# Rudrabha/Wav2Lip

Measured on AMD Instinct MI355X. Metric: face-frames/sec (96x96, mel T=16), higher is better.
Workload: dtype f32

## Files before the change

include/w2l_hip.h:

```cpp
#ifndef W2L_HIP_H
#define W2L_HIP_H

#include <stddef.h>
#include <stdint.h>

#ifdef __cplusplus
extern "C" {
#endif

#define W2L_OK 0
#define W2L_ERR_ARG (-1)
#define W2L_ERR_HIP (-2)
#define W2L_ERR_NOMEM (-3)

#define W2L_ACT_NONE 0
#define W2L_ACT_RELU 1
#define W2L_ACT_SIGMOID 2
#define W2L_ACT_LEAKY 3

#define W2L_PREC_F32 0
#define W2L_PREC_BF16 1

const char* w2l_last_error(void);
int w2l_abi_version(void);
// ... 198 lines not shown
int w2l_thin1x1_dgrad_bf16(void* stream, long long npix, int cin, int cout, const void* dz, int dz_cs, const float* w,
                           const void* res, int res_cs, void* dx, int dx_cs);
int w2l_thin1x1_wgrad_bf16(void* stream, long long npix, int cin, int cout, const void* x, int x_cs, const void* dz, int dz_cs,
                           float* dweight, float* dbias);
int w2l_thin1x1_wgrad_blocks(long long npix);
int w2l_nchw_to_nhwc_bf16(void* stream, int N, int C, int H, int W, const float* x, void* y, int y_cs, int c_zero_to);
int w2l_nhwc_bf16_to_nchw(void* stream, int N, int C, int H, int W, const void* x, int x_cs, float* y);


int w2l_bn_train_stats(void* stream, long long rows, int C, const float* z, int z_cs, const float* gamma,
                       const float* beta, float eps, float momentum, float* running_mean, float* running_var,
                       float* mean, float* rstd, float* scale, float* shift);
int w2l_affine_act(void* stream, long long rows, int C, const float* z, int z_cs, const float* scale,
                   const float* shift, const float* res, int res_cs, int act, float* y, int y_cs);
int w2l_bn_train_bwd(void* stream, long long rows, int C, const float* dy, int dy_cs, const float* y, int y_cs,
                     const float* z, int z_cs, int act, const float* mean, const float* rstd, const float* scale,
                     float* dgamma, float* dbeta, float* dz, int dz_cs, float* g_out, int g_cs);
int w2l_act_bwd(void* stream, long long rows, int C, const float* dy, int dy_cs, const float* y, int y_cs, int act,
                const float* scale, float* dz, int dz_cs, float* g_out, int g_cs);
int w2l_add_rows(void* stream, long long rows, int C, const float* a, int a_cs, const float* b, int b_cs, float* out,
                 int out_cs);
int w2l_col_sum(void* stream, long long rows, int C, const float* x, int x_cs, float* out);

int w2l_l1_mean(void* stream, long long n, const float* a, const float* b, float* loss_out);
int w2l_l1_bwd(void* stream, long long n, const float* a, const float* b, const float* gout, float* da);
int w2l_cosine_bce_bwd(void* stream, int N, int C, const float* a, const float* v, const float* y, const float* gout,
                       float* da, float* dv);
int w2l_l2norm_bwd(void* stream, int N, int C, const float* x, int x_cs, const float* dy, float* dx, int dx_cs);
int w2l_bce_bwd(void* stream, int N, const float* p, const float* y, const float* gout, float* dp);

int w2l_shifted_pdist(void* stream, int T, int C, int vshift, const float* f1, const float* f2, float* out);

typedef struct {
    uint64_t frames, mel;
    int32_t T, start;
    int32_t pad[2];
} w2l_sync_row;
typedef struct {
    int32_t row0, n;
} w2l_lse_segment;

int w2l_sync_window_rows(void* stream, int B, const w2l_sync_row* rows, int S, float* face_in, int face_cs, float* mel_in,
                         int mel_cs);
int w2l_lse_score_segments(void* stream, int n_seg, const w2l_lse_segment* segs, int C, int vshift, const float* face_emb,
                           const float* audio_emb, float* mdist, float* scores);

typedef struct w2l_adam_tensor {
    float* param;
    const float* grad;
    float* exp_avg;
    float* exp_avg_sq;
    long long n;
} w2l_adam_tensor;
typedef struct w2l_adam w2l_adam_t;
int w2l_adam_create(int ntensors, const long long* sizes_host, w2l_adam_t** out);
int w2l_adam_destroy(w2l_adam_t* h);
int w2l_adam_step(w2l_adam_t* h, void* stream, const w2l_adam_tensor* tensors_host, float lr, float beta1, float beta2,
                  float eps, float weight_decay, int step);


typedef struct w2l_plan w2l_plan_t;
int w2l_plan_create(w2l_plan_t** out);
int w2l_plan_destroy(w2l_plan_t* p);
int w2l_plan_add_conv(w2l_plan_t* p, const w2l_conv_t* c, int N, int H, int W, const float* x, int x_cs,
                      float* y, int y_cs, const float* res, int res_cs);
int w2l_plan_add_convb(w2l_plan_t* p, const w2l_convb_t* c, int N, int H, int W, const void* x, int x_cs, void* y, int y_cs,
                       const void* res, int res_cs, const float* scale, const float* shift);
int w2l_plan_add_convb_head(w2l_plan_t* p, const w2l_convb_t* c, int N, int H, int W, const void* x, int x_cs, uint8_t* frames,
                            float* y32, int y32_cs, const float* scale, const float* shift);
int w2l_plan_copy_item(w2l_plan_t* dst, const w2l_plan_t* src, int index);
int w2l_plan_run(const w2l_plan_t* p, void* stream);
int w2l_plan_size(const w2l_plan_t* p);
int w2l_plan_autotune(w2l_plan_t* p, void* stream, int reps);
int w2l_plan_get_config(const w2l_plan_t* p, int index, int* tile, int* ksplit);
int w2l_plan_set_config(w2l_plan_t* p, int index, int tile, int ksplit);
int w2l_plan_executed_flops(const w2l_plan_t* p, long long* flops_out, int* config_out);
int w2l_conv_num_igemm_tiles(void);
int w2l_flops_begin(void);
long long w2l_flops_end(long long* by_family);
int w2l_clock_probe(void* stream, int spin_us, unsigned long long* out2_dev);
int w2l_conv_config_family(int id);
int w2l_conv_exclude_families(int mask);
int w2l_igemm_block_order(int order, int order_r, int tiles_m, int tiles_n, int nphase, int* out);
int w2l_plan_profile(const w2l_plan_t* p, void* stream, int reps, float* ms_out);

#define W2L_TUNE_KEY_INTS 17
int w2l_tune_key_ints(void);
int w2l_tune_set(const int* key, int tile, int ksplit);
int w2l_tune_entry_applicable(const int* key, int tile);
int w2l_tune_clear(void);
int w2l_tune_count(void);
int w2l_tune_export(int* out, int cap_entries);

#ifdef __cplusplus
}
#endif
#endif
```

wav2lip_amd/_lib.py:

```python
import ctypes as C
import os

_HERE = os.path.dirname(os.path.abspath(__file__))
LIB_PATH = os.environ.get("W2L_HIP_LIB") or os.path.join(_HERE, "lib", "libw2l_hip.so")

ACT_NONE, ACT_RELU, ACT_SIGMOID, ACT_LEAKY = 0, 1, 2, 3
PREC_F32, PREC_BF16 = 0, 1


class ConvGeom(C.Structure):
    _fields_ = [(n, C.c_int) for n in
                ("transposed", "cin", "cout", "kh", "kw", "sh", "sw", "ph", "pw", "oph", "opw", "act")]


class AdamTensor(C.Structure):
    _fields_ = [("param", C.c_void_p), ("grad", C.c_void_p), ("exp_avg", C.c_void_p), ("exp_avg_sq", C.c_void_p),
                ("n", C.c_longlong)]


class WgradInfo(C.Structure):
    _fields_ = [(n, C.c_int) for n in ("family", "cfg", "ksplit", "chunk", "K", "kstep", "reduce_blocks")]


class WgradBf16Info(C.Structure):
# ... 72 lines not shown
    "w2l_mel_create": (_i, [_vp, _vp, C.POINTER(_vp)]),
    "w2l_mel_destroy": (_i, [_vp]),
    "w2l_mel_num_frames": (_i, [_ll]),
    "w2l_melspectrogram": (_i, [_vp, _vp, _vp, _ll, _vp]),
    "w2l_mel_stream_cols": (_i, [_vp, _vp, _vp, _i, _vp, _i]),
    "w2l_mel_gather": (_i, [_vp, _vp, _i, _vp, _i, _vp, _i, _i]),
    "w2l_mel_gather_bf16": (_i, [_vp, _vp, _i, _vp, _i, _vp, _i, _i]),
    "w2l_mel_gather_rows": (_i, [_vp, _vp, _i, _vp, _i, _i]),
    "w2l_mel_gather_rows_bf16": (_i, [_vp, _vp, _i, _vp, _i, _i]),
    "w2l_resample_sinc": (_i, [_vp, _vp, _i, _vp, _i, C.c_double, _vp, _vp, _i, _i, _vp]),
    "w2l_l2norm_rows": (_i, [_vp, _i, _i, _vp, _i, _vp]),
    "w2l_cosine_bce": (_i, [_vp, _i, _i, _vp, _vp, _vp, _vp, _vp]),
    "w2l_bce_mean": (_i, [_vp, _i, _vp, _vp, _vp]),
    "w2l_conv_update": (_i, [_vp, _vp, _vp, _vp, _vp]),
    "w2l_conv_wgrad": (_i, [C.POINTER(ConvGeom), _vp, _i, _i, _i, _vp, _i, _vp, _i, _vp]),
    "w2l_conv_wgrad_prec": (_i, [C.POINTER(ConvGeom), _vp, _i, _i, _i, _vp, _i, _vp, _i, _vp, _i]),
    "w2l_conv_wgrad_resolve": (_i, [C.POINTER(ConvGeom), _i, _i, _i, _i, _i, _i, C.POINTER(WgradInfo)]),
    "w2l_conv_wgrad_set_cfg": (_i, [_i, _i]),
    "w2l_wgrad_divmod_host": (_i, [_i, _i, _vp, _vp, _vp, _vp]),
    "w2l_convb_create": (_i, [C.POINTER(ConvGeom), _vp, _vp, C.POINTER(_vp)]),
    "w2l_convb_update": (_i, [_vp, _vp, _vp]),
    "w2l_convb_update_many": (_i, [_i, _vp, _vp, _vp]),
    "w2l_convb_destroy": (_i, [_vp]),
    "w2l_convb_forward": (_i, [_vp, _vp, _i, _i, _i, _vp, _i, _vp, _i, _vp, _i, _vp, _vp, _i]),
    "w2l_convb_attach_head": (_i, [_vp, _vp, _vp, _vp, _i, _i, _vp]),
    "w2l_convb_forward_head": (_i, [_vp, _vp, _i, _i, _i, _vp, _i, _vp, _vp, _i, _vp, _vp]),
    "w2l_convb_forward_bn": (_i, [_vp, _vp, _i, _i, _i, _vp, _i, _vp, _i, _vp, _vp, _vp, _f, _f, _vp, _vp, _vp, _vp, _vp, _vp]),
    "w2l_convb_forward_bnbwd": (_i, [_vp, _vp, _i, _i, _i, _vp, _i, _vp, _i, _vp, _i, _vp, _i, _vp, _i, _i, _vp, _vp, _vp, _vp, _vp, _vp,
                                     C.POINTER(C.c_int)]),
    "w2l_convb_forward_actbwd": (_i, [_vp, _vp, _i, _i, _i, _vp, _i, _vp, _i, _vp, _i, _vp, _i, _i, _vp, C.POINTER(C.c_int)]),
    "w2l_convb_set_tile": (_i, [_vp, _i]),
    "w2l_convb_num_tiles": (_i, []),
    "w2l_convb_resolve": (_i, [_vp, _i, _i, _i, _i, C.POINTER(C.c_int), C.POINTER(C.c_int), C.POINTER(C.c_int)]),
    "w2l_conv_wgrad_bf16": (_i, [C.POINTER(ConvGeom), _vp, _i, _i, _i, _vp, _i, _vp, _i, _vp]),
    "w2l_conv_wgrad_bf16_resolve": (_i, [C.POINTER(ConvGeom), _i, _i, _i, _i, _i, C.POINTER(WgradBf16Info)]),
    "w2l_bn_train_stats_bf16": (_i, [_vp, _ll, _i, _i, _vp, _i, _vp, _vp, _f, _f, _vp, _vp, _vp, _vp, _vp, _vp]),
    "w2l_affine_act_bf16": (_i, [_vp, _ll, _i, _vp, _i, _vp, _vp, _vp, _i, _i, _vp, _i]),
    "w2l_bn_train_bwd_bf16": (_i, [_vp, _ll, _i, _i, _vp, _i, _vp, _i, _vp, _i, _i, _vp, _vp, _vp, _vp, _vp, _vp, _vp, _i, _vp, _i]),
    "w2l_bn_train_bwd_apply_bf16": (_i, [_vp, _ll, _i, _vp, _i, _vp, _i, _vp, _i, _i, _vp, _vp, _vp, _vp, _vp, _vp, _vp, _i, _vp, _i]),
    "w2l_act_bwd_bf16": (_i, [_vp, _ll, _i, _vp, _i, _vp, _i, _i, _vp, _vp, _i, _vp, _i]),
    "w2l_add_rows_bf16": (_i, [_vp, _ll, _i, _vp, _i, _vp, _i, _vp, _i]),
    "w2l_col_sum_bf16": (_i, [_vp, _ll, _i, _vp, _i, _vp]),
    "w2l_thin1x1_forward_bf16": (_i, [_vp, _ll, _i, _i, _vp, _i, _vp, _vp, _i, _vp, _i]),
    "w2l_thin1x1_dgrad_bf16": (_i, [_vp, _ll, _i, _i, _vp, _i, _vp, _vp, _i, _vp, _i]),
    "w2l_thin1x1_wgrad_bf16": (_i, [_vp, _ll, _i, _i, _vp, _i, _vp, _i, _vp, _vp]),
    "w2l_thin1x1_wgrad_blocks": (_i, [_ll]),
    "w2l_nchw_to_nhwc_bf16": (_i, [_vp, _i, _i, _i, _i, _vp, _vp, _i, _i]),
    "w2l_nhwc_bf16_to_nchw": (_i, [_vp, _i, _i, _i, _i, _vp, _i, _vp]),
    "w2l_bn_train_stats": (_i, [_vp, _ll, _i, _vp, _i, _vp, _vp, _f, _f, _vp, _vp, _vp, _vp, _vp, _vp]),
    "w2l_affine_act": (_i, [_vp, _ll, _i, _vp, _i, _vp, _vp, _vp, _i, _i, _vp, _i]),
    "w2l_bn_train_bwd": (_i, [_vp, _ll, _i, _vp, _i, _vp, _i, _vp, _i, _i, _vp, _vp, _vp, _vp, _vp, _vp, _i, _vp, _i]),
    "w2l_act_bwd": (_i, [_vp, _ll, _i, _vp, _i, _vp, _i, _i, _vp, _vp, _i, _vp, _i]),
    "w2l_add_rows": (_i, [_vp, _ll, _i, _vp, _i, _vp, _i, _vp, _i]),
    "w2l_col_sum": (_i, [_vp, _ll, _i, _vp, _i, _vp]),
    "w2l_l1_mean": (_i, [_vp, _ll, _vp, _vp, _vp]),
    "w2l_l1_bwd": (_i, [_vp, _ll, _vp, _vp, _vp, _vp]),
    "w2l_cosine_bce_bwd": (_i, [_vp, _i, _i, _vp, _vp, _vp, _vp, _vp, _vp]),
    "w2l_l2norm_bwd": (_i, [_vp, _i, _i, _vp, _i, _vp, _vp, _i]),
    "w2l_bce_bwd": (_i, [_vp, _i, _vp, _vp, _vp, _vp]),
    "w2l_shifted_pdist": (_i, [_vp, _i, _i, _i, _vp, _vp, _vp]),
    "w2l_sync_window_rows": (_i, [_vp, _i, _vp, _i, _vp, _i, _vp, _i]),
    "w2l_lse_score_segments": (_i, [_vp, _i, _vp, _i, _i, _vp, _vp, _vp, _vp]),
    "w2l_adam_create": (_i, [_i, C.POINTER(_ll), C.POINTER(_vp)]),
    "w2l_adam_destroy": (_i, [_vp]),
    "w2l_adam_step": (_i, [_vp, _vp, C.POINTER(AdamTensor), _f, _f, _f, _f, _f, _i]),
    "w2l_plan_create": (_i, [C.POINTER(_vp)]),
    "w2l_plan_destroy": (_i, [_vp]),
    "w2l_plan_add_conv": (_i, [_vp, _vp, _i, _i, _i, _vp, _i, _vp, _i, _vp, _i]),
    "w2l_plan_add_convb": (_i, [_vp, _vp, _i, _i, _i, _vp, _i, _vp, _i, _vp, _i, _vp, _vp]),
    "w2l_plan_add_convb_head": (_i, [_vp, _vp, _i, _i, _i, _vp, _i, _vp, _vp, _i, _vp, _vp]),
    "w2l_plan_copy_item": (_i, [_vp, _vp, _i]),
    "w2l_plan_run": (_i, [_vp, _vp]),
    "w2l_plan_size": (_i, [_vp]),
    "w2l_plan_autotune": (_i, [_vp, _vp, _i]),
    "w2l_plan_get_config": (_i, [_vp, _i, C.POINTER(_i), C.POINTER(_i)]),
    "w2l_plan_set_config": (_i, [_vp, _i, _i, _i]),
    "w2l_plan_profile": (_i, [_vp, _vp, _i, _vp]),
    "w2l_plan_executed_flops": (_i, [_vp, C.POINTER(_ll), C.POINTER(_i)]),
    "w2l_conv_num_igemm_tiles": (_i, []),
    "w2l_flops_begin": (_i, []),
    "w2l_flops_end": (_ll, [C.POINTER(_ll)]),
    "w2l_clock_probe": (C.c_int, [C.c_void_p, C.c_int, C.c_void_p]),
    "w2l_igemm_block_order": (C.c_int, [C.c_int, C.c_int, C.c_int, C.c_int, C.c_int, C.c_void_p]),
    "w2l_conv_config_family": (_i, [_i]),
    "w2l_conv_exclude_families": (_i, [_i]),
    "w2l_tune_key_ints": (_i, []),
    "w2l_tune_set": (_i, [C.POINTER(_i), _i, _i]),
    "w2l_tune_entry_applicable": (_i, [C.POINTER(_i), _i]),
    "w2l_tune_clear": (_i, []),
    "w2l_tune_count": (_i, []),
    "w2l_tune_export": (_i, [C.POINTER(_i), _i]),
}

_lib = None

TUNE_TABLE_PATH = os.path.join(_HERE, "tune_table.json")
EXACT = os.environ.get("W2L_EXACT", "0") == "1"
EXACT_TABLE_PATH = os.path.join(_HERE, "tune_table_exact.json")
FAMILY_NAMES = ("igemm", "wino", "wino2", "tp2", "wino4", "split", "wino2s", "tp2s", "stem7s", "k3s")
SPLIT_FAMILIES = frozenset(FAMILY_NAMES.index(n) for n in ("split", "wino2s", "tp2s", "stem7s", "k3s"))
FAMILY_WINO4, FAMILY_SPLIT, FAMILY_WINO2S, FAMILY_TP2S, FAMILY_STEM7S, FAMILY_K3S = (
    FAMILY_NAMES.index(n) for n in ("wino4", "split", "wino2s", "tp2s", "stem7s", "k3s"))


def config_ids(lib, family):
    f = FAMILY_NAMES.index(family)
    return [i for i in range(lib.w2l_conv_num_tiles()) if lib.w2l_conv_config_family(i) == f]


NO_SPLIT = os.environ.get("W2L_SPLIT", "1") == "0"
NOSPLIT_TABLE_PATH = os.path.join(_HERE, "tune_table_nosplit.json")


def load_tune_table(lib, path=None):
    import json
    if path is None and NO_SPLIT and not EXACT and not os.environ.get("W2L_TUNE_TABLE"):
        return load_tune_table(lib, TUNE_TABLE_PATH) + load_tune_table(lib, NOSPLIT_TABLE_PATH)
    path = path or os.environ.get("W2L_TUNE_TABLE") or (EXACT_TABLE_PATH if EXACT else TUNE_TABLE_PATH)
    if path == "0" or not os.path.exists(path):
        return 0
    with open(path) as fh:
        doc = json.load(fh)
    nk = lib.w2l_tune_key_ints()
    if doc.get("key_ints") != nk or doc.get("num_configs", 0) > lib.w2l_conv_num_tiles():
        raise RuntimeError("tune table %s was written for another library build (key_ints %s / configs %s)"
                           % (path, doc.get("key_ints"), doc.get("num_configs")))
    n = 0
    for e in doc["entries"]:
        key = (C.c_int * nk)(*e[:nk])
        check_rc = lib.w2l_tune_set(key, int(e[nk]), int(e[nk + 1]))
        if check_rc != 0:
            raise RuntimeError("tune table %s: bad entry %s" % (path, e))
        n += 1
    return n


def export_tune_table(lib):
    nk = lib.w2l_tune_key_ints()
    n = lib.w2l_tune_count()
    buf = (C.c_int * (max(n, 1) * (nk + 2)))()
    n = lib.w2l_tune_export(buf, n)
    return sorted([int(buf[i * (nk + 2) + j]) for j in range(nk + 2)] for i in range(n))


def save_tune_table(lib, path, note=""):
    import json
    nk = lib.w2l_tune_key_ints()
    for e in export_tune_table(lib):
        if not lib.w2l_tune_entry_applicable((C.c_int * nk)(*e[:nk]), e[nk]):
            raise RuntimeError("tune table entry %s names a configuration its shape cannot run" % e)
    doc = {"key_ints": lib.w2l_tune_key_ints(), "num_configs": lib.w2l_conv_num_tiles(),
           "key": "transposed cin cout kh kw sh sw ph pw oph opw precision has_residual head_c N H W -> config ksplit",
           "note": note, "entries": export_tune_table(lib)}
    with open(path, "w") as fh:
        fh.write(json.dumps(doc, indent=None, separators=(",", ":")).replace("],[", "],\n[") + "\n")
    return len(doc["entries"])


def load():
    global _lib
    if _lib is not None:
        return _lib
    import torch
    if not os.path.exists(LIB_PATH):
        raise RuntimeError(
            "wav2lip_amd: HIP library %s is missing; build it with `make -C wav2lip_amd/csrc` "
# ... 28 lines not shown
```

wav2lip_amd/csrc/conv_wino4.hip:

```cpp
#include "w2l_common.h"
#include "w2l_pk.h"

namespace w2l {

typedef float f32x16 __attribute__((ext_vector_type(16)));
typedef unsigned int u32x4 __attribute__((ext_vector_type(4)));

__device__ __forceinline__ f32x2 pk2_mul4(f32x2 a) {
    f32x2 d;
    asm("v_pk_mul_f32 %0, %1, 4.0 op_sel_hi:[1,0]" : "=v"(d) : "v"(a));
    return d;
}

template <int BLK>
__device__ __forceinline__ void w4_at3(f32x2 m0, f32x2 m1, f32x2 m2, f32x2& o0, f32x2& o1, f32x2& o2, f32x2& o3) {
    if (BLK == 0) {
        const f32x2 sm = pk2_add(m1, m2);
        o1 = pk2_sub(m1, m2);
        o0 = pk2_add(m0, sm);
        o2 = sm;
        o3 = o1;
    } else {
        const f32x2 sm = pk2_add(m0, m1);
        const f32x2 df = pk2_sub(m0, m1);
        o0 = sm;
        o1 = pk2_add(df, df);
        o2 = pk2_mul4(sm);
        o3 = pk2_add(pk2_mul4(o1), m2);
    }
}

template <int PI, int PJ, int LDY>
__device__ __forceinline__ void w4_partial_store(const f32x16 (&acc)[9], const int r, float* y, const int tstride) {
    f32x2 R[4][3];
#pragma unroll
    for (int jl = 0; jl < 3; ++jl) {
        const f32x2 m0 = {acc[0 + jl][r], acc[0 + jl][r + 1]};
        const f32x2 m1 = {acc[3 + jl][r], acc[3 + jl][r + 1]};
        const f32x2 m2 = {acc[6 + jl][r], acc[6 + jl][r + 1]};
        w4_at3<PI>(m0, m1, m2, R[0][jl], R[1][jl], R[2][jl], R[3][jl]);
    }
    f32x2 P1[4];
#pragma unroll
    for (int oa = 0; oa < 4; ++oa) {
        f32x2 P[4];
        if (PI == 0 && oa == 3) {
#pragma unroll
            for (int ob = 0; ob < 4; ++ob) P[ob] = P1[ob];
        } else {
            w4_at3<PJ>(R[oa][0], R[oa][1], R[oa][2], P[0], P[1], P[2], P[3]);
        }
        if (oa == 1) {
#pragma unroll
            for (int ob = 0; ob < 4; ++ob) P1[ob] = P[ob];
        }
        float* yo = y + (oa * 4) * LDY;
#pragma unroll
        for (int ob = 0; ob < 4; ++ob) {
            yo[ob * LDY] = P[ob].x;
            yo[ob * LDY + tstride] = P[ob].y;
        }
    }
}

#ifndef W4_DBG
#define W4_DBG 0
#endif
#ifdef W4_TRACE
__device__ unsigned long long w4_trace_buf[256 * 16 * 8];
__device__ unsigned long long w4_trace_rt[256 * 16 * 2];
#define W4_STAMP(k)                                                                                              \
    do {                                                                                                         \
        if (threadIdx.x == 0 && trace_item < 16) {                                                               \
            w4_trace_buf[(blockIdx.x * 16 + trace_item) * 8 + (k)] = __builtin_readcyclecounter();              \
            if ((k) == 0 || (k) == 7)                                                                            \
                w4_trace_rt[(blockIdx.x * 16 + trace_item) * 2 + ((k) ? 1 : 0)] = __builtin_amdgcn_s_memrealtime(); \
        }                                                                                                        \
    } while (0)
#else
#define W4_STAMP(k)
#endif

constexpr unsigned kW4Oob = 0x80000000u;
constexpr int kW4BT = 32;
constexpr int kW4BC = 64;
constexpr int kW4KS = 8;
constexpr int kW4LDK = kW4KS + 4;
constexpr int kW4VPOS = kW4BT * kW4LDK;
constexpr int kW4VBUF = 36 * kW4VPOS;
constexpr int kW4NRAW = 3;
constexpr int kW4RAW4 = 512 * kW4NRAW;
constexpr int kW4PS = 186;
constexpr int kW4QS = 4 * kW4PS;
static_assert(2 * kW4QS <= kW4RAW4 && kW4PS % 8 == 2 && kW4QS % 16 == 8, "raw plane geometry");
constexpr int kW4LDY = kW4BC + 4;
constexpr int kW4LdsFloats = 2 * kW4VBUF + 2 * kW4RAW4 * 4;
constexpr int kW4LdsBytes = kW4LdsFloats * 4 + 2 * kW4BT * 4;
static_assert(4 * kW4BT * 4 * kW4LDY <= kW4LdsFloats, "one round of the four partial staging tiles must fit");
static_assert(kW4LdsBytes <= 160 * 1024, "LDS budget");

struct Wino4KArgs {
    const float* x;
    float* y;
    const float* res;
    const float* u;
    const float* scale;
    const float* shift;
    int N, H, W, cin, x_cs;
    int cout, y_cs, res_cs;
    int TH, TW;
    int bh, bw, ni;
    int nby, nbx, ngi;
    int RH, RW, R4;
    int pitch, istride;
    float inv_rw, inv_rh;
    int nks;
    int tiles_n;
    long long total;
    int act;
};

__global__ __launch_bounds__(512, 2) void conv_wino4_f32_kernel(const Wino4KArgs a) {
    extern __shared__ __attribute__((aligned(16))) char smem[];
    float* Vs = reinterpret_cast<float*>(smem);
    float* Rs = Vs + 2 * kW4VBUF;
    int* s_opix = reinterpret_cast<int*>(Rs + 2 * kW4RAW4 * 4);
    int* s_oflag = s_opix + kW4BT;

    const __amdgpu_buffer_rsrc_t rx = __builtin_amdgcn_make_buffer_rsrc(
        const_cast<float*>(a.x), 0, (int)((((long long)a.N * a.H * a.W - 1) * a.x_cs + a.cin) * 4), 0x00020000);

    const unsigned total = (unsigned)a.total;
    const unsigned per = (total + 7u) / 8u;
    const unsigned xcd = blockIdx.x & 7u, gw = gridDim.x >> 3;
#ifdef W4_TRACE
    int trace_item = -1;
#endif
    for (unsigned jw = blockIdx.x >> 3; jw < per; jw += gw) {
    const unsigned bid = xcd * per + jw;
    if (bid >= total) break;
#ifdef W4_TRACE
    ++trace_item;
#endif
    W4_STAMP(0);
    int t = threadIdx.x;
    asm volatile("" : "+v"(t));
    const int lane = t & 63;
    const int wave = __builtin_amdgcn_readfirstlane(t >> 6);
    const int wn = wave & 1;
    const int pb = wave >> 1;
    const int PI = pb >> 1, PJ = pb & 1;
    const int tile_n = (int)(bid % (unsigned)a.tiles_n);
    unsigned mb = bid / (unsigned)a.tiles_n;
    const int bx_i = (int)(mb % (unsigned)a.nbx);
    mb /= (unsigned)a.nbx;
    const int by_i = (int)(mb % (unsigned)a.nby);
    const int gi = (int)(mb / (unsigned)a.nby);
    const int n0 = tile_n * kW4BC;
    const int bhw = a.bh * a.bw;

    if (t < kW4BT) {
        const int il = t / bhw, r = t - il * bhw;
        const int tyl = r / a.bw, txl = r - tyl * a.bw;
        const int n = gi * a.ni + il, ty = by_i * a.bh + tyl, tx = bx_i * a.bw + txl;
        int o = -1, f = 0;
        if (il < a.ni && n < a.N && ty < a.TH && tx < a.TW) {
            o = (n * a.H + 4 * ty) * a.W + 4 * tx;
#pragma unroll
            for (int k = 0; k < 4; ++k) f |= ((4 * ty + k < a.H) ? (1 << k) : 0) | ((4 * tx + k < a.W) ? (16 << k) : 0);
        }
        s_opix[t] = o;
        s_oflag[t] = f;
    }

    unsigned goff[kW4NRAW];
    int rst[kW4NRAW];
#pragma unroll
    for (int k = 0; k < kW4NRAW; ++k) {
        const int e = t + 512 * k;
        const int q = (e >> 3) & 1, pix = (e >> 4) * 8 + (e & 7);
        unsigned off = kW4Oob;
        int st = -1;
        if (pix < a.R4) {
            const int p2 = (int)(((float)pix + 0.5f) * a.inv_rw);
            const int rxx = pix - p2 * a.RW;
            const int il = (int)(((float)p2 + 0.5f) * a.inv_rh);
            const int ry = p2 - il * a.RH;
            st = (q * kW4QS + (rxx & 3) * kW4PS + il * a.istride + ry * a.pitch + (rxx >> 2)) * 16;
            const int n = gi * a.ni + il;
            const int iy = 4 * by_i * a.bh - 1 + ry, ix = 4 * bx_i * a.bw - 1 + rxx;
            if (n < a.N && (unsigned)iy < (unsigned)a.H && (unsigned)ix < (unsigned)a.W)
                off = ((unsigned)((n * a.H + iy) * a.W + ix) * (unsigned)a.x_cs + (unsigned)(q * 4)) * 4u;
        }
        goff[k] = off;
        rst[k] = st;
    }
    f32x4 rawreg[kW4NRAW];
    auto raw_gload = [&](int step) {
        const unsigned soff = (unsigned)(step * kW4KS * 4);
#pragma unroll
        for (int k = 0; k < kW4NRAW; ++k)
            rawreg[k] = __builtin_bit_cast(f32x4, __builtin_amdgcn_raw_buffer_load_b128(rx, (int)goff[k], (int)soff, 0));
    };
    auto raw_store = [&](int buf) {
        char* dst = reinterpret_cast<char*>(Rs) + buf * (kW4RAW4 * 16);
#pragma unroll
        for (int k = 0; k < kW4NRAW; ++k)
            if (rst[k] >= 0) *reinterpret_cast<f32x4*>(dst + rst[k]) = rawreg[k];
    };

    const bool tf_wave = wave < 6;
    const int q = lane & 1;
    int ra, rb, rc, rd;
    float ca, cb, cc;
    switch (wave) {
        case 0: ra = 0; ca = 0.f; rb = 0; cb = 4.f; rc = 2; cc = -5.f; rd = 4; break;
        case 1: ra = 1; ca = -4.f; rb = 2; cb = -4.f; rc = 3; cc = 1.f; rd = 4; break;
        case 2: ra = 1; ca = 4.f; rb = 2; cb = -4.f; rc = 3; cc = -1.f; rd = 4; break;
        case 3: ra = 1; ca = -2.f; rb = 2; cb = -1.f; rc = 3; cc = 2.f; rd = 4; break;
        case 4: ra = 1; ca = 2.f; rb = 2; cb = -1.f; rc = 3; cc = -2.f; rd = 4; break;
        default: ra = 1; ca = 0.f; rb = 1; cb = 4.f; rc = 3; cc = -5.f; rd = 5; break;
    }
    int tf_base;
    {
        const int tl = lane >> 1;
        const int il = tl / bhw, r = tl - il * bhw;
        const int tyl = r / a.bw, txl = r - tyl * a.bw;
        const int ilc = il < a.ni ? il : 0;
        tf_base = (q * kW4QS + ilc * a.istride + 4 * tyl * a.pitch + txl) * 16;
    }
    const int rp = a.pitch * 16;
    const int o_a = tf_base + ra * rp, o_b = tf_base + rb * rp, o_c = tf_base + rc * rp, o_d = tf_base + rd * rp;
    float* const vwr = Vs + ((wave < 6 ? wave : 0) * 6) * kW4VPOS + (lane >> 1) * kW4LDK + q * 4;
    f32x4 rr[6];
    auto tf_rows = [&](int buf, int c0) {
        const char* src = reinterpret_cast<const char*>(Rs) + buf * (kW4RAW4 * 16);
#pragma unroll
        for (int c = c0; c < c0 + 1; ++c) {
            const int co = ((c & 3) * kW4PS + (c >> 2)) * 16;
            const f32x4 va = *reinterpret_cast<const f32x4*>(src + o_a + co), vb = *reinterpret_cast<const f32x4*>(src + o_b + co);
            const f32x4 vc = *reinterpret_cast<const f32x4*>(src + o_c + co), vd = *reinterpret_cast<const f32x4*>(src + o_d + co);
#pragma unroll
            for (int e = 0; e < 4; ++e) rr[c][e] = fmaf(ca, va[e], fmaf(cb, vb[e], fmaf(cc, vc[e], vd[e])));
        }
    };
    auto tf_cols_store = [&](int buf) {
        float* dst = vwr + buf * kW4VBUF;
        f32x4 v0, v1, v2, v3, v4, v5;
#pragma unroll
        for (int e = 0; e < 4; ++e) {
            const float p = fmaf(-4.f, rr[2][e], rr[4][e]);
            const float qq = fmaf(4.f, rr[1][e], -rr[3][e]);
            const float p2 = rr[4][e] - rr[2][e];
            const float q2 = 2.f * (rr[3][e] - rr[1][e]);
            v0[e] = fmaf(4.f, rr[0][e], fmaf(-5.f, rr[2][e], rr[4][e]));
            v1[e] = p - qq;
            v2[e] = p + qq;
            v3[e] = p2 + q2;
            v4[e] = p2 - q2;
            v5[e] = fmaf(4.f, rr[1][e], fmaf(-5.f, rr[3][e], rr[5][e]));
        }
        *reinterpret_cast<f32x4*>(dst + 0 * kW4VPOS) = v0;
        *reinterpret_cast<f32x4*>(dst + 1 * kW4VPOS) = v1;
        *reinterpret_cast<f32x4*>(dst + 2 * kW4VPOS) = v2;
        *reinterpret_cast<f32x4*>(dst + 3 * kW4VPOS) = v3;
        *reinterpret_cast<f32x4*>(dst + 4 * kW4VPOS) = v4;
        *reinterpret_cast<f32x4*>(dst + 5 * kW4VPOS) = v5;
    };

    const int nb = (n0 >> 5) + wn;
    const int F = a.nks * 36;
    const __amdgpu_buffer_rsrc_t ru = __builtin_amdgcn_make_buffer_rsrc(
        const_cast<float*>(a.u + (long long)nb * F * 256), 0, F * 1024, 0x00020000);
    const unsigned bl_lane = (unsigned)(lane * 16);
    const int pos0 = 18 * PI + 3 * PJ;
    const unsigned bl_pb = (unsigned)pos0 * 1024u;
    auto bload = [&](int kc, int s) {
        const unsigned soff = (unsigned)kc * 36864u + bl_pb + (unsigned)(6 * (s / 3) + (s % 3)) * 1024u;
        return __builtin_bit_cast(f32x4, __builtin_amdgcn_raw_buffer_load_b128(ru, (int)bl_lane, (int)soff, 0));
    };
    constexpr int RING = 3;
    f32x4 bq[RING];

    f32x16 acc[9];
#pragma unroll
    for (int s = 0; s < 9; ++s)
#pragma unroll
        for (int r = 0; r < 16; ++r) acc[s][r] = 0.f;

    const int nsteps = a.cin / kW4KS;
    raw_gload(0);
#pragma unroll
    for (int i = 0; i < RING; ++i) bq[i] = bload(0, i);
    raw_store(0);
    raw_gload(1);
    __syncthreads();
    W4_STAMP(1);
    if (tf_wave) {
#pragma unroll
        for (int c = 0; c < 6; ++c) tf_rows(0, c);
        tf_cols_store(0);
    }
    raw_store(1);
    __syncthreads();
    W4_STAMP(2);

    const float* Abase = Vs + pos0 * kW4VPOS + (lane & 31) * kW4LDK + (lane >> 5) * 4;
    for (int step = 0; step < nsteps; ++step) {
        const int buf = step & 1;
        const float* Ab = Abase + buf * kW4VBUF;
        f32x4 af = *reinterpret_cast<const f32x4*>(Ab);
#pragma unroll
        for (int s = 0; s < 9; ++s) {
            const f32x4 ac = af;
            if (s < 8) af = *reinterpret_cast<const f32x4*>(Ab + (6 * ((s + 1) / 3) + ((s + 1) % 3)) * kW4VPOS);
            const f32x4 bc = bq[s % RING];
#if !(W4_DBG & 8)
            bq[s % RING] = (s < 9 - RING) ? bload(step, s + RING) : bload(step + 1, s + RING - 9);
#endif
// ... 62 lines not shown
                w4_partial_store<0, 0, kW4LDY>(acc, 4 * round + 2, yrow + 2 * TS, TS);
            } else if (pb == 1) {
                w4_partial_store<0, 1, kW4LDY>(acc, 4 * round, yrow, TS);
                w4_partial_store<0, 1, kW4LDY>(acc, 4 * round + 2, yrow + 2 * TS, TS);
            } else if (pb == 2) {
                w4_partial_store<1, 0, kW4LDY>(acc, 4 * round, yrow, TS);
                w4_partial_store<1, 0, kW4LDY>(acc, 4 * round + 2, yrow + 2 * TS, TS);
            } else {
                w4_partial_store<1, 1, kW4LDY>(acc, 4 * round, yrow, TS);
                w4_partial_store<1, 1, kW4LDY>(acc, 4 * round + 2, yrow + 2 * TS, TS);
            }
        }
        __syncthreads();
#pragma unroll
        for (int i = 0; i < NIT; ++i) {
            const int id = i * 512 + t;
            const int pix = out_pix(round, i);
            const bool ok = pix >= 0;
            const f32x4 rvv = rv[i];
            const float* src = Ys + (id / CG) * kW4LDY + c4 * 4;
            const f32x4 p0 = *reinterpret_cast<const f32x4*>(src);
            const f32x4 p1 = *reinterpret_cast<const f32x4*>(src + kPart);
            const f32x4 p2 = *reinterpret_cast<const f32x4*>(src + 2 * kPart);
            const f32x4 p3 = *reinterpret_cast<const f32x4*>(src + 3 * kPart);
            f32x4 v;
#pragma unroll
            for (int e = 0; e < 4; ++e) {
                const float xv = fmaf((p0[e] + p1[e]) + (p2[e] + p3[e]), sc[e], sh[e]) + rvv[e];
                v[e] = fmaf(neg_slope, fminf(xv, 0.f), fmaxf(xv, 0.f));
            }
            __builtin_amdgcn_raw_buffer_store_b128(
                __builtin_bit_cast(u32x4, v), ry, (int)(ok ? ((unsigned)pix * (unsigned)a.y_cs + (unsigned)ch) * 4u : kW4Oob), 0, 0);
        }
        if (round < 3) res_load(round + 1);
        __syncthreads();
        W4_STAMP(4 + round);
    }
    }
}

struct Wino4PackArgs {
    const float* w;
    float* u;
    int cin, cout;
    int transposed;
};

__global__ void wino4_pack_kernel(const Wino4PackArgs a) {
    const int total = a.cout * a.cin;
    const int nks = a.cin / 8;
    constexpr double G[6][3] = {{0.25, 0.0, 0.0},          {-1.0 / 6, -1.0 / 6, -1.0 / 6}, {-1.0 / 6, 1.0 / 6, -1.0 / 6},
                                {1.0 / 24, 1.0 / 12, 1.0 / 6}, {1.0 / 24, -1.0 / 12, 1.0 / 6}, {0.0, 0.0, 1.0}};
    for (int j = blockIdx.x * blockDim.x + threadIdx.x; j < total; j += gridDim.x * blockDim.x) {
        const int e = j & 3, n = (j >> 2) & 31, h = (j >> 7) & 1;
        const int blk = j >> 8;
        const int kc = blk % nks, nbk = blk / nks;
        const int co = nbk * 32 + n;
        const int ci = kc * 8 + 4 * h + e;
        const float* g = a.transposed ? a.w + ((long long)ci * a.cout + co) * 9 : a.w + ((long long)co * a.cin + ci) * 9;
        double gd[3][3];
#pragma unroll
        for (int aa = 0; aa < 3; ++aa)
#pragma unroll
            for (int bb = 0; bb < 3; ++bb) gd[aa][bb] = (double)(a.transposed ? g[(2 - aa) * 3 + (2 - bb)] : g[aa * 3 + bb]);
        float* dst = a.u + (long long)blk * 36 * 256 + (j & 255);
#pragma unroll
        for (int pi = 0; pi < 6; ++pi)
#pragma unroll
            for (int pj = 0; pj < 6; ++pj) {
                double sum = 0.0;
#pragma unroll
                for (int aa = 0; aa < 3; ++aa)
#pragma unroll
                    for (int bb = 0; bb < 3; ++bb) sum += G[pi][aa] * gd[aa][bb] * G[pj][bb];
                dst[(pi * 6 + pj) * 256] = (float)sum;
            }
    }
}

struct W4Block { int bh, bw, ni; };
static const W4Block kW4Blocks[] = {{4, 8, 1}, {8, 4, 1}, {4, 4, 2}, {2, 8, 2}, {8, 2, 1}, {2, 4, 3}, {4, 2, 3}, {3, 3, 3},
                                    {2, 2, 6}, {2, 3, 4}, {3, 2, 4}, {1, 4, 6}, {4, 1, 5}, {1, 2, 10}, {2, 1, 9}, {1, 1, 15}};

static bool wino4_block_fits(const W4Block& b) {
    const int RH = 4 * b.bh + 2, RW = 4 * b.bw + 2;
    return b.bh * b.bw * b.ni <= kW4BT && b.ni * RH * RW * 2 <= kW4RAW4 && b.ni * RH * (b.bw + 1) <= kW4PS;
}

static void wino4_plane_geom(const W4Block& b, int* pitch, int* istride) {
    static const int kGroup[2][16] = {{0, 1, 2, 3, 12, 13, 14, 15, 20, 21, 22, 23, 24, 25, 26, 27},
                                      {4, 5, 6, 7, 8, 9, 10, 11, 16, 17, 18, 19, 28, 29, 30, 31}};
    const int RH = 4 * b.bh + 2, bhw = b.bh * b.bw;
    int best = 1 << 30;
    *pitch = b.bw + 1;
    *istride = RH * (b.bw + 1);
    for (int p = b.bw + 1; p <= b.bw + 4; ++p)
        for (int is = RH * p; is <= RH * p + 15; ++is) {
            if (b.ni * is > kW4PS) break;
            int cost = (p - b.bw - 1) + (is - RH * p);
            for (int g = 0; g < 4; ++g) {
                int cnt[16] = {0};
                for (int k = 0; k < 16; ++k) {
                    const int lane = kGroup[g & 1][k] + 32 * (g >> 1);
                    const int tl = lane >> 1, q = lane & 1;
                    const int il = tl / bhw, r = tl % bhw;
                    const int ilc = il < b.ni ? il : 0;
                    ++cnt[(q * kW4QS + ilc * is + 4 * (r / b.bw) * p + r % b.bw) & 15];
                }
                for (int k = 0; k < 16; ++k) cost += cnt[k] > 1 ? (cnt[k] - 1) * 64 * cnt[k] : 0;
            }
            if (cost < best) { best = cost; *pitch = p; *istride = is; }
        }
}

static W4Block wino4_pick_block(int N, int TH, int TW) {
    W4Block best = {1, 1, 1};
    double best_cost = 1e300;
    for (const W4Block& b : kW4Blocks) {
        if (!wino4_block_fits(b)) continue;
        const double items = (double)ceil_div(TH, b.bh) * ceil_div(TW, b.bw) * ceil_div(N, b.ni);
        const double halo = (double)(4 * b.bh + 2) * (4 * b.bw + 2) / (16.0 * b.bh * b.bw);
        const double cost = items * (1.0 + 0.05 * halo);
        if (cost < best_cost) { best_cost = cost; best = b; }
    }
    return best;
}

bool wino4_ok(int cin, int cout) { return cin % kW4KS == 0 && cout % kW4BC == 0; }

long long wino4_u_floats(int cin, int cout) { return (long long)cout * cin * 36; }

int wino4_pack(const float* w, float* u, int cin, int cout, int transposed, hipStream_t stream) {
    Wino4PackArgs pa;
    pa.w = w; pa.u = u; pa.cin = cin; pa.cout = cout; pa.transposed = transposed;
    long long blocks = ((long long)cin * cout + 255) / 256;
    if (blocks > 8192) blocks = 8192;
    hipLaunchKernelGGL(wino4_pack_kernel, dim3((unsigned)blocks), dim3(256), 0, stream, pa);
    W2L_HIP_CHECK(hipGetLastError());
    return W2L_OK;
}

int wino4_init_attrs() {
    static bool done = false;
    if (done) return W2L_OK;
    W2L_HIP_CHECK(hipFuncSetAttribute(reinterpret_cast<const void*>(conv_wino4_f32_kernel),
                                      hipFuncAttributeMaxDynamicSharedMemorySize, kW4LdsBytes));
    done = true;
    return W2L_OK;
}

int wino4_launch(const WinoKArgs& w, const float* u4, hipStream_t stream, long long* flops_out) {
    Wino4KArgs a;
    a.x = w.x; a.y = w.y; a.res = w.res; a.u = u4; a.scale = w.scale; a.shift = w.shift;
    a.N = w.N; a.H = w.H; a.W = w.W; a.cin = w.cin; a.x_cs = w.x_cs;
    a.cout = w.cout; a.y_cs = w.y_cs; a.res_cs = w.res_cs; a.act = w.act;
    a.TH = (a.H + 3) / 4;
    a.TW = (a.W + 3) / 4;
    const W4Block b = wino4_pick_block(a.N, a.TH, a.TW);
    a.bh = b.bh; a.bw = b.bw; a.ni = b.ni;
    a.nby = ceil_div(a.TH, b.bh);
    a.nbx = ceil_div(a.TW, b.bw);
    a.ngi = ceil_div(a.N, b.ni);
    a.RH = 4 * b.bh + 2;
    a.RW = 4 * b.bw + 2;
    a.R4 = b.ni * a.RH * a.RW;
    wino4_plane_geom(b, &a.pitch, &a.istride);
    a.inv_rw = 1.0f / (float)a.RW;
    a.inv_rh = 1.0f / (float)a.RH;
    a.nks = a.cin / 8;
    a.tiles_n = a.cout / kW4BC;
    a.total = (long long)a.ngi * a.nby * a.nbx * a.tiles_n;
    W2L_REQUIRE(a.total < (1ll << 31), "grid too large");
    W2L_REQUIRE((long long)a.N * a.H * a.W < (1ll << 31), "tensor too large");
    if (flops_out) {
        *flops_out = 2ll * 36 * a.total * kW4BT * kW4BC * a.cin;
        return W2L_OK;
    }
    long long grid = (a.total + 7) / 8 * 8;
    if (grid > 256) grid = 256;
    hipLaunchKernelGGL(conv_wino4_f32_kernel, dim3((unsigned)grid), dim3(512), kW4LdsBytes, stream, a);
    W2L_HIP_CHECK(hipGetLastError());
    return W2L_OK;
}

}

#ifdef W4_TRACE
extern "C" int w2l_dbg_w4_trace(unsigned long long* out) {
    if (hipMemcpyFromSymbol(out, HIP_SYMBOL(w2l::w4_trace_buf), sizeof(w2l::w4_trace_buf)) != hipSuccess) return 1;
    return (int)hipMemcpyFromSymbol(out + 256 * 16 * 8, HIP_SYMBOL(w2l::w4_trace_rt), sizeof(w2l::w4_trace_rt));
}
#endif
```

Measured before the change: 29350.

## Add segmented full-width row blocking to Winograd F(4,3) conv kernel

Adds a second work decomposition for the wino4 kernel. Each block takes a run of consecutive full-width tile rows across image boundaries, up to 8 segments, instead of a rectangular bh x bw x ni block. The host picks the segmented mode when its estimated cost (block count weighted by halo overhead) beats the rectangular one, and chooses pitch and pad to limit LDS bank conflicts. The intent is to cut padding waste and halo reloads for small images such as 24x24 tiles. In exchange the raw LDS plane grows and per-pixel address computation adds a segment lookup loop.

```diff
diff --git a/include/w2l_hip.h b/include/w2l_hip.h
--- a/include/w2l_hip.h
+++ b/include/w2l_hip.h
@@ -304,6 +304,7 @@
 int w2l_conv_config_family(int id);
 int w2l_conv_exclude_families(int mask);
 int w2l_igemm_block_order(int order, int order_r, int tiles_m, int tiles_n, int nphase, int* out);
+int w2l_wino4_block_plan(int N, int H, int W, int* out);
 int w2l_plan_profile(const w2l_plan_t* p, void* stream, int reps, float* ms_out);
 
 #define W2L_TUNE_KEY_INTS 17
diff --git a/wav2lip_amd/_lib.py b/wav2lip_amd/_lib.py
--- a/wav2lip_amd/_lib.py
+++ b/wav2lip_amd/_lib.py
@@ -178,6 +178,7 @@
     "w2l_flops_end": (_ll, [C.POINTER(_ll)]),
     "w2l_clock_probe": (C.c_int, [C.c_void_p, C.c_int, C.c_void_p]),
     "w2l_igemm_block_order": (C.c_int, [C.c_int, C.c_int, C.c_int, C.c_int, C.c_int, C.c_void_p]),
+    "w2l_wino4_block_plan": (_i, [_i, _i, _i, _vp]),
     "w2l_conv_config_family": (_i, [_i]),
     "w2l_conv_exclude_families": (_i, [_i]),
     "w2l_tune_key_ints": (_i, []),
diff --git a/wav2lip_amd/csrc/conv_wino4.hip b/wav2lip_amd/csrc/conv_wino4.hip
--- a/wav2lip_amd/csrc/conv_wino4.hip
+++ b/wav2lip_amd/csrc/conv_wino4.hip
@@ -90,12 +90,15 @@
 constexpr int kW4VBUF = 36 * kW4VPOS;
 constexpr int kW4NRAW = 3;
 constexpr int kW4RAW4 = 512 * kW4NRAW;
-constexpr int kW4PS = 186;
+constexpr int kW4PS = 202;
 constexpr int kW4QS = 4 * kW4PS;
-static_assert(2 * kW4QS <= kW4RAW4 && kW4PS % 8 == 2 && kW4QS % 16 == 8, "raw plane geometry");
+constexpr int kW4RAWB = 2 * kW4QS;
+static_assert(kW4RAWB >= kW4RAW4 && kW4PS % 8 == 2 && kW4QS % 16 == 8, "raw plane geometry");
 constexpr int kW4LDY = kW4BC + 4;
-constexpr int kW4LdsFloats = 2 * kW4VBUF + 2 * kW4RAW4 * 4;
-constexpr int kW4LdsBytes = kW4LdsFloats * 4 + 2 * kW4BT * 4;
+constexpr int kW4LdsFloats = 2 * kW4VBUF + 2 * kW4RAWB * 4;
+constexpr int kW4S = 8;
+constexpr int kW4SegInts = 8;
+constexpr int kW4LdsBytes = kW4LdsFloats * 4 + 2 * kW4BT * 4 + kW4S * kW4SegInts * 4;
 static_assert(4 * kW4BT * 4 * kW4LDY <= kW4LdsFloats, "one round of the four partial staging tiles must fit");
 static_assert(kW4LdsBytes <= 160 * 1024, "LDS budget");
 
@@ -110,6 +113,8 @@
     int cout, y_cs, res_cs;
     int TH, TW;
     int bh, bw, ni;
+    int seg_r, seg_pad;
+    int units;
     int nby, nbx, ngi;
     int RH, RW, R4;
     int pitch, istride;
@@ -120,12 +125,14 @@
     int act;
 };
 
+template <bool SEG>
 __global__ __launch_bounds__(512, 2) void conv_wino4_f32_kernel(const Wino4KArgs a) {
     extern __shared__ __attribute__((aligned(16))) char smem[];
     float* Vs = reinterpret_cast<float*>(smem);
     float* Rs = Vs + 2 * kW4VBUF;
-    int* s_opix = reinterpret_cast<int*>(Rs + 2 * kW4RAW4 * 4);
+    int* s_opix = reinterpret_cast<int*>(Rs + 2 * kW4RAWB * 4);
     int* s_oflag = s_opix + kW4BT;
+    int* s_seg = s_oflag + kW4BT;
 
     const __amdgpu_buffer_rsrc_t rx = __builtin_amdgcn_make_buffer_rsrc(
         const_cast<float*>(a.x), 0, (int)((((long long)a.N * a.H * a.W - 1) * a.x_cs + a.cin) * 4), 0x00020000);
@@ -158,8 +165,38 @@
     const int gi = (int)(mb / (unsigned)a.nby);
     const int n0 = tile_n * kW4BC;
     const int bhw = a.bh * a.bw;
-
-    if (t < kW4BT) {
+    const int u0 = (int)(bid / (unsigned)a.tiles_n) * a.seg_r;
+    const int u1 = min(u0 + a.seg_r, a.units);
+    const int nfirst = SEG ? u0 / a.TH : 0;
+
+    if (SEG) {
+        if (t < kW4S) {
+            const int n = nfirst + t;
+            const int ua = max(u0, n * a.TH), ub = min(u1, (n + 1) * a.TH);
+            const int row0 = ua - u0;
+            int* sg = s_seg + t * kW4SegInts;
+            sg[0] = n;
+            sg[1] = ua - n * a.TH;
+            sg[2] = max(ub - ua, 0);
+            sg[3] = 4 * row0 + 2 * t;
+            sg[4] = (4 * row0 + 2 * t) * a.pitch + t * a.seg_pad;
+            sg[5] = row0 * a.TW;
+        }
+        if (t < kW4BT) {
+            const int r = t / a.TW, txl = t - r * a.TW;
+            const int u = u0 + r;
+            int o = -1, f = 0;
+            if (u < u1) {
+                const int n = u / a.TH, ty = u - n * a.TH;
+                o = (n * a.H + 4 * ty) * a.W + 4 * txl;
+#pragma unroll
+                for (int k = 0; k < 4; ++k) f |= ((4 * ty + k < a.H) ? (1 << k) : 0) | ((4 * txl + k < a.W) ? (16 << k) : 0);
+            }
+            s_opix[t] = o;
+            s_oflag[t] = f;
+        }
+        __syncthreads();
+    } else if (t < kW4BT) {
         const int il = t / bhw, r = t - il * bhw;
         const int tyl = r / a.bw, txl = r - tyl * a.bw;
         const int n = gi * a.ni + il, ty = by_i * a.bh + tyl, tx = bx_i * a.bw + txl;
@@ -181,7 +218,22 @@
         const int q = (e >> 3) & 1, pix = (e >> 4) * 8 + (e & 7);
         unsigned off = kW4Oob;
         int st = -1;
-        if (pix < a.R4) {
+        if (SEG) {
+            const int p2 = (int)(((float)pix + 0.5f) * a.inv_rw);
+            const int rxx = pix - p2 * a.RW;
+            int j = 0;
+#pragma unroll
+            for (int sgi = 1; sgi < kW4S; ++sgi)
+                if (s_seg[sgi * kW4SegInts + 2] > 0 && p2 >= s_seg[sgi * kW4SegInts + 3]) j = sgi;
+            const int* sg = s_seg + j * kW4SegInts;
+            const int ry = p2 - sg[3];
+            if (ry < 4 * sg[2] + 2) {
+                st = (q * kW4QS + (rxx & 3) * kW4PS + sg[4] + ry * a.pitch + (rxx >> 2)) * 16;
+                const int iy = 4 * sg[1] - 1 + ry, ix = rxx - 1;
+                if ((unsigned)iy < (unsigned)a.H && (unsigned)ix < (unsigned)a.W)
+                    off = ((unsigned)((sg[0] * a.H + iy) * a.W + ix) * (unsigned)a.x_cs + (unsigned)(q * 4)) * 4u;
+            }
+        } else if (pix < a.R4) {
             const int p2 = (int)(((float)pix + 0.5f) * a.inv_rw);
             const int rxx = pix - p2 * a.RW;
             const int il = (int)(((float)p2 + 0.5f) * a.inv_rh);
@@ -203,7 +255,7 @@
             rawreg[k] = __builtin_bit_cast(f32x4, __builtin_amdgcn_raw_buffer_load_b128(rx, (int)goff[k], (int)soff, 0));
     };
     auto raw_store = [&](int buf) {
-        char* dst = reinterpret_cast<char*>(Rs) + buf * (kW4RAW4 * 16);
+        char* dst = reinterpret_cast<char*>(Rs) + buf * (kW4RAWB * 16);
 #pragma unroll
         for (int k = 0; k < kW4NRAW; ++k)
             if (rst[k] >= 0) *reinterpret_cast<f32x4*>(dst + rst[k]) = rawreg[k];
@@ -222,7 +274,13 @@
         default: ra = 1; ca = 0.f; rb = 1; cb = 4.f; rc = 3; cc = -5.f; rd = 5; break;
     }
     int tf_base;
-    {
+    if (SEG) {
+        const int tl = lane >> 1;
+        int r = tl / a.TW, txl = tl - r * a.TW;
+        if (u0 + r >= u1) r = 0, txl = 0;
+        const int j = (u0 + r) / a.TH - nfirst;
+        tf_base = (q * kW4QS + (4 * r + 2 * j) * a.pitch + j * a.seg_pad + txl) * 16;
+    } else {
         const int tl = lane >> 1;
         const int il = tl / bhw, r = tl - il * bhw;
         const int tyl = r / a.bw, txl = r - tyl * a.bw;
@@ -234,7 +292,7 @@
     float* const vwr = Vs + ((wave < 6 ? wave : 0) * 6) * kW4VPOS + (lane >> 1) * kW4LDK + q * 4;
     f32x4 rr[6];
     auto tf_rows = [&](int buf, int c0) {
-        const char* src = reinterpret_cast<const char*>(Rs) + buf * (kW4RAW4 * 16);
+        const char* src = reinterpret_cast<const char*>(Rs) + buf * (kW4RAWB * 16);
 #pragma unroll
         for (int c = c0; c < c0 + 1; ++c) {
             const int co = ((c & 3) * kW4PS + (c >> 2)) * 16;
@@ -463,9 +521,10 @@
 static const W4Block kW4Blocks[] = {{4, 8, 1}, {8, 4, 1}, {4, 4, 2}, {2, 8, 2}, {8, 2, 1}, {2, 4, 3}, {4, 2, 3}, {3, 3, 3},
                                     {2, 2, 6}, {2, 3, 4}, {3, 2, 4}, {1, 4, 6}, {4, 1, 5}, {1, 2, 10}, {2, 1, 9}, {1, 1, 15}};
 
+constexpr int kW4RectCells = 186;
 static bool wino4_block_fits(const W4Block& b) {
     const int RH = 4 * b.bh + 2, RW = 4 * b.bw + 2;
-    return b.bh * b.bw * b.ni <= kW4BT && b.ni * RH * RW * 2 <= kW4RAW4 && b.ni * RH * (b.bw + 1) <= kW4PS;
+    return b.bh * b.bw * b.ni <= kW4BT && b.ni * RH * RW * 2 <= kW4RAW4 && b.ni * RH * (b.bw + 1) <= kW4RectCells;
 }
 
 static void wino4_plane_geom(const W4Block& b, int* pitch, int* istride) {
@@ -477,7 +536,7 @@
     *istride = RH * (b.bw + 1);
     for (int p = b.bw + 1; p <= b.bw + 4; ++p)
         for (int is = RH * p; is <= RH * p + 15; ++is) {
-            if (b.ni * is > kW4PS) break;
+            if (b.ni * is > kW4RectCells) break;
             int cost = (p - b.bw - 1) + (is - RH * p);
             for (int g = 0; g < 4; ++g) {
                 int cnt[16] = {0};
@@ -494,7 +553,7 @@
         }
 }
 
-static W4Block wino4_pick_block(int N, int TH, int TW) {
+static W4Block wino4_pick_block(int N, int TH, int TW, double* cost_out) {
     W4Block best = {1, 1, 1};
     double best_cost = 1e300;
     for (const W4Block& b : kW4Blocks) {
@@ -504,7 +563,62 @@
         const double cost = items * (1.0 + 0.05 * halo);
         if (cost < best_cost) { best_cost = cost; best = b; }
     }
+    *cost_out = best_cost;
     return best;
+}
+
+struct W4Seg { int R, pitch, pad, nblk; double cost; };
+
+static int wino4_seg_count(int off, int R, int TH) { return (off + R - 1) / TH + 1; }
+
+static int wino4_seg_worst(int R, int TH, int nblk) {
+    int worst = 1;
+    for (int b = 0; b < nblk && b < TH; ++b) worst = std::max(worst, wino4_seg_count((b * R) % TH, R, TH));
+    return worst;
+}
+
+static int wino4_seg_conflicts(int R, int TH, int TW, int nblk, int pitch, int pad) {
+    static const int kGroup[2][16] = {{0, 1, 2, 3, 12, 13, 14, 15, 20, 21, 22, 23, 24, 25, 26, 27},
+                                      {4, 5, 6, 7, 8, 9, 10, 11, 16, 17, 18, 19, 28, 29, 30, 31}};
+    int cost = 0;
+    for (int b = 0; b < nblk && b < TH; ++b) {
+        const int off = (b * R) % TH;
+        for (int g = 0; g < 4; ++g) {
+            int cnt[16] = {0};
+            for (int k = 0; k < 16; ++k) {
+                const int lane = kGroup[g & 1][k] + 32 * (g >> 1);
+                const int tl = lane >> 1, q = lane & 1;
+                int r = tl / TW, c = tl % TW;
+                if (r >= R) r = 0, c = 0;
+                const int j = (off + r) / TH;
+                ++cnt[(q * kW4QS + (4 * r + 2 * j) * pitch + j * pad + c) & 15];
+            }
+            for (int k = 0; k < 16; ++k) cost += cnt[k] > 1 ? (cnt[k] - 1) * 64 * cnt[k] : 0;
+        }
+    }
+    return cost;
+}
+
+static W4Seg wino4_pick_seg(int N, int TH, int TW) {
+    W4Seg s = {0, 0, 0, 0, 1e300};
+    const int units = N * TH, RW = 4 * TW + 2;
+    for (int R = std::min(kW4BT / TW, units); R >= 1; --R) {
+        const int nblk = ceil_div(units, R);
+        const int ns = wino4_seg_worst(R, TH, nblk), rows = 4 * R + 2 * ns;
+        if (ns > kW4S || rows * RW * 2 > kW4RAW4 || rows * (TW + 1) > kW4PS) continue;
+        s.R = R;
+        s.nblk = nblk;
+        s.cost = (double)nblk * (1.0 + 0.05 * (double)(rows * RW) / (16.0 * R * TW));
+        int best = 1 << 30;
+        for (int p = TW + 1; p <= TW + 4; ++p)
+            for (int pad = 0; pad < 8; ++pad) {
+                if (rows * p + (ns - 1) * pad > kW4PS) break;
+                const int c = wino4_seg_conflicts(R, TH, TW, nblk, p, pad) + (p - TW - 1) + pad;
+                if (c < best) { best = c; s.pitch = p; s.pad = pad; }
+            }
+        break;
+    }
+    return s;
 }
 
 bool wino4_ok(int cin, int cout) { return cin % kW4KS == 0 && cout % kW4BC == 0; }
@@ -524,7 +638,9 @@
 int wino4_init_attrs() {
     static bool done = false;
     if (done) return W2L_OK;
-    W2L_HIP_CHECK(hipFuncSetAttribute(reinterpret_cast<const void*>(conv_wino4_f32_kernel),
+    W2L_HIP_CHECK(hipFuncSetAttribute(reinterpret_cast<const void*>(conv_wino4_f32_kernel<false>),
+                                      hipFuncAttributeMaxDynamicSharedMemorySize, kW4LdsBytes));
+    W2L_HIP_CHECK(hipFuncSetAttribute(reinterpret_cast<const void*>(conv_wino4_f32_kernel<true>),
                                       hipFuncAttributeMaxDynamicSharedMemorySize, kW4LdsBytes));
     done = true;
     return W2L_OK;
@@ -537,20 +653,37 @@
     a.cout = w.cout; a.y_cs = w.y_cs; a.res_cs = w.res_cs; a.act = w.act;
     a.TH = (a.H + 3) / 4;
     a.TW = (a.W + 3) / 4;
-    const W4Block b = wino4_pick_block(a.N, a.TH, a.TW);
-    a.bh = b.bh; a.bw = b.bw; a.ni = b.ni;
-    a.nby = ceil_div(a.TH, b.bh);
-    a.nbx = ceil_div(a.TW, b.bw);
-    a.ngi = ceil_div(a.N, b.ni);
-    a.RH = 4 * b.bh + 2;
-    a.RW = 4 * b.bw + 2;
-    a.R4 = b.ni * a.RH * a.RW;
-    wino4_plane_geom(b, &a.pitch, &a.istride);
-    a.inv_rw = 1.0f / (float)a.RW;
-    a.inv_rh = 1.0f / (float)a.RH;
+    W2L_REQUIRE((long long)a.N * a.TH < (1ll << 30), "grid too large");
+    double rect_cost;
+    const W4Block b = wino4_pick_block(a.N, a.TH, a.TW, &rect_cost);
+    const W4Seg sg = wino4_pick_seg(a.N, a.TH, a.TW);
+    const bool seg = sg.R > 0 && sg.cost < rect_cost;
     a.nks = a.cin / 8;
     a.tiles_n = a.cout / kW4BC;
-    a.total = (long long)a.ngi * a.nby * a.nbx * a.tiles_n;
+    a.units = a.N * a.TH;
+    if (seg) {
+        a.bh = a.bw = a.ni = a.nby = a.nbx = 1;
+        a.ngi = sg.nblk;
+        a.seg_r = sg.R; a.seg_pad = sg.pad;
+        a.RH = 0;
+        a.RW = 4 * a.TW + 2;
+        a.R4 = 0;
+        a.pitch = sg.pitch; a.istride = 0;
+        a.total = (long long)sg.nblk * a.tiles_n;
+    } else {
+        a.bh = b.bh; a.bw = b.bw; a.ni = b.ni;
+        a.seg_r = 0; a.seg_pad = 0;
+        a.nby = ceil_div(a.TH, b.bh);
+        a.nbx = ceil_div(a.TW, b.bw);
+        a.ngi = ceil_div(a.N, b.ni);
+        a.RH = 4 * b.bh + 2;
+        a.RW = 4 * b.bw + 2;
+        a.R4 = b.ni * a.RH * a.RW;
+        wino4_plane_geom(b, &a.pitch, &a.istride);
+        a.total = (long long)a.ngi * a.nby * a.nbx * a.tiles_n;
+    }
+    a.inv_rw = 1.0f / (float)a.RW;
+    a.inv_rh = a.RH ? 1.0f / (float)a.RH : 0.f;
     W2L_REQUIRE(a.total < (1ll << 31), "grid too large");
     W2L_REQUIRE((long long)a.N * a.H * a.W < (1ll << 31), "tensor too large");
     if (flops_out) {
@@ -559,11 +692,35 @@
     }
     long long grid = (a.total + 7) / 8 * 8;
     if (grid > 256) grid = 256;
-    hipLaunchKernelGGL(conv_wino4_f32_kernel, dim3((unsigned)grid), dim3(512), kW4LdsBytes, stream, a);
+    if (seg)
+        hipLaunchKernelGGL(conv_wino4_f32_kernel<true>, dim3((unsigned)grid), dim3(512), kW4LdsBytes, stream, a);
+    else
+        hipLaunchKernelGGL(conv_wino4_f32_kernel<false>, dim3((unsigned)grid), dim3(512), kW4LdsBytes, stream, a);
     W2L_HIP_CHECK(hipGetLastError());
     return W2L_OK;
 }
 
+}
+
+extern "C" int w2l_wino4_block_plan(int N, int H, int W, int* out) {
+    using namespace w2l;
+    W2L_REQUIRE(out && N >= 1 && H >= 1 && W >= 1 && (long long)N * ((H + 3) / 4) < (1ll << 30), "wino4_block_plan: bad arguments");
+    const int TH = (H + 3) / 4, TW = (W + 3) / 4;
+    double rect_cost;
+    const W4Block b = wino4_pick_block(N, TH, TW, &rect_cost);
+    const W4Seg sg = wino4_pick_seg(N, TH, TW);
+    const bool seg = sg.R > 0 && sg.cost < rect_cost;
+    int pitch = sg.pitch, istride = 0;
+    if (!seg) wino4_plane_geom(b, &pitch, &istride);
+    out[0] = seg;
+    out[1] = seg ? sg.nblk : ceil_div(TH, b.bh) * ceil_div(TW, b.bw) * ceil_div(N, b.ni);
+    out[2] = seg ? sg.R : b.bh;
+    out[3] = seg ? TW : b.bw;
+    out[4] = seg ? 0 : b.ni;
+    out[5] = pitch;
+    out[6] = seg ? sg.pad : istride;
+    out[7] = kW4PS;
+    return W2L_OK;
 }
 
 #ifdef W4_TRACE
```

After: 29950 (median of 6 runs). 2.0% higher.
